# bxlab/bx-python

Measured on AMD Instinct MI355X. Metric: M overlap-queries/s at 100M x 10M intervals (count-only), higher is better.
Workload: dtype int32

## Files before the change

### bx-python_amd/csrc/count_dense.hpp

```cpp
#pragma once
#include "offset_cells.hpp"

namespace bxmi {

constexpr int BD_UNIT_LOG2 = 19;
constexpr int BD_RSHIFT = 19;
constexpr int BD_MARGIN = 8192;
constexpr int BD_MAX_F = 6;
constexpr int BD_MAX_SHIFT = 19;
constexpr int BD_OV_MAX = 32704;
constexpr int BD_TABLE_FROM_FIRST = 2, BD_TABLE_FROM_LAST = 6;
constexpr int BD_THREADS = 1024;
constexpr int BD_LONG_SLOTS = 64;
constexpr int BD_LONG_CAP = 320;
constexpr int BD_HDR_QS = 6;

struct BdLayout {
    int nce, ncs;
    int bitsE, bitsS, metaE, metaS, hdr, ov, bytes;
    int ov_cap;
};

__host__ __device__ inline BdLayout bd_layout(int unit_log2)
{
// ... 917 lines not shown
    {
        const int nl = s_nlong < BD_LONG_CAP ? s_nlong : BD_LONG_CAP;
        for (int k = 0; k < nl; k++) {
            const uint2 lr = s_long[k];
            const unsigned first = lr.x, end = lr.x + lr.y;
            const unsigned q0 = first >> 2, nq4 = ((end + 3u) >> 2) - q0;
            for (unsigned q = threadIdx.x; q < nq4; q += BD_THREADS) {
                const unsigned idx4 = q0 + q;
                bd_answer_slot<FMT, QB, EXP, W8>(I, out, idx4, bd_valid_mask(4u * idx4, first, end), reinterpret_cast<const bd_v4u *>(recs)[idx4]);
            }
        }
    }
}

constexpr int BW_MASK_WORDS = 128;
constexpr int BW_PF = 9;
constexpr unsigned BW_IDLE = 0xFFFFFFFFu;
#ifndef BW_EXP
#define BW_EXP 0
#endif
#ifndef BW_B
#define BW_B 64
#endif
#ifndef BS_UNROLL
#define BS_UNROLL 1
#endif

__device__ __forceinline__ unsigned bw_wave_inclusive_sum(unsigned v)
{
    v += (unsigned)__builtin_amdgcn_update_dpp(0, (int)v, 0x111, 0xf, 0xf, false);
    v += (unsigned)__builtin_amdgcn_update_dpp(0, (int)v, 0x112, 0xf, 0xf, false);
    v += (unsigned)__builtin_amdgcn_update_dpp(0, (int)v, 0x114, 0xf, 0xf, false);
    v += (unsigned)__builtin_amdgcn_update_dpp(0, (int)v, 0x118, 0xf, 0xf, false);
    v += (unsigned)__builtin_amdgcn_update_dpp(0, (int)v, 0x142, 0xa, 0xf, false);
    v += (unsigned)__builtin_amdgcn_update_dpp(0, (int)v, 0x143, 0xc, 0xf, false);
    return v;
}

template <bool RAW = false>
__device__ __forceinline__ void bp_count_slot(const BdImage &I, bd_v4u v, unsigned (&c)[4])
{
    const unsigned rec[4] = {v.x, v.y, v.z, v.w};
    unsigned relE[4], relS[4];
    unsigned long long cellE[4], cellS[4];
#pragma unroll
    for (int j = 0; j < 4; j++) {
// ... 170 lines not shown
    } else {
        bd_v2u o;
        o.x = c[0] | (c[1] << 16), o.y = c[2] | (c[3] << 16);
        reinterpret_cast<bd_v2u *>(out)[idx4] = o;
    }
}

template <bool W8, int DEPTH, bool WIDE = false, int THREADS = BD_THREADS, bool TOT = false>
__global__ __launch_bounds__(THREADS) void bw_search_kernel(const BmSeg *__restrict__ segs, const int4 *__restrict__ items,
                                                               const int *__restrict__ n_items, const unsigned short *__restrict__ unitT, int64_t ntp,
                                                               const unsigned *__restrict__ recs ,
                                                               unsigned short *__restrict__ out , int tile_log2,
                                                               const unsigned *__restrict__ gate, unsigned *__restrict__ xcd_next ,
                                                               unsigned long long *__restrict__ total_slots = nullptr )
{
    if (gate && *gate == 0) return;
    extern __shared__ __attribute__((aligned(16))) int32_t dyn[];
    __shared__ long long s_red[TOT ? THREADS / 64 : 1];
    unsigned long long acc = 0ull;
    int acc_seg = -1;
    constexpr int LONG_CAP = THREADS == BD_THREADS ? BD_LONG_CAP : BD_LONG_CAP / 2;
    constexpr int PF = THREADS == BD_THREADS ? BW_PF : 10;
    __shared__ uint2 s_long[LONG_CAP];
    __shared__ int s_nlong, s_next, s_item_next;
    __shared__ __attribute__((aligned(8))) unsigned s_mask[THREADS / 64][BW_MASK_WORDS];
    const int nit = *n_items;
    const int per_xcd = (nit + 7) >> 3;
    const int xcd = (int)(blockIdx.x & 7);
    const int it_lo = xcd * per_xcd, it_hi = it_lo + per_xcd < nit ? it_lo + per_xcd : nit;
    const int lane = lane_id(), wave = __builtin_amdgcn_readfirstlane((int)(threadIdx.x >> 6));
    unsigned *const wmask = s_mask[wave];
    wmask[lane] = 0u, wmask[64 + lane] = 0u;
    if (threadIdx.x == 0) s_item_next = it_lo + (int)atomicAdd(&xcd_next[xcd], 1u);
    __syncthreads();
    int it = __builtin_amdgcn_readfirstlane(s_item_next);
    __syncthreads();
    const unsigned tile_slots = ((1u << tile_log2) + (unsigned)BM_PAD_ROOM) >> 2;
    while (it < it_hi) {
        const int4 item = items[it];
        const int unit = item.x & 0xffff, t0 = item.y, t1 = item.z;
        const BmSeg &sg = segs[item.x >> 16];
        if (TOT && (item.x >> 16) != acc_seg) {
            if (acc_seg >= 0) {
                block_accumulate_i64((long long)acc, s_red, total_slots + (int64_t)acc_seg * PT_SLOTS + (blockIdx.x & (PT_SLOTS - 1)));
                __syncthreads();
            }
// ... 38 lines not shown
#pragma unroll
            for (int k = 0; k < PF; k++) {
                const int i = k * THREADS + (int)threadIdx.x;
                if (i < n4) reinterpret_cast<bm_v4i *>(dyn)[i] = v[k];
            }
        }
        __syncthreads();
        const int it_nx = __builtin_amdgcn_readfirstlane(s_item_next);
        BdImage I;
        {
            unsigned char *base = reinterpret_cast<unsigned char *>(dyn);
            I.img16 = (lds_u16_p) reinterpret_cast<unsigned short *>(base);
            I.cE = (lds_cell_p) reinterpret_cast<unsigned long long *>(base + LP.cellsE);
            I.cS = (lds_cell_p) reinterpret_cast<unsigned long long *>(base + LP.cellsS);
            const unsigned *hdr = reinterpret_cast<const unsigned *>(base + LP.hdr);
            I.eLo = (int)hdr[0], I.sLo = (int)hdr[1];
            I.bias = I.sLo - I.eLo;
            I.lo = (long long)((unsigned long long)hdr[2] | ((unsigned long long)hdr[3] << 32));
            I.s_ord = sg.ix.s_ord, I.e_sorted = sg.e_sorted;
            I.off_mask = (1u << (g.shift + g.f)) - 1u;
            I.img8 = (lds_u8_p)base;
            I.rshift = g.rshift, I.cell_log2 = cell_log2, I.cell_mask = (1u << cell_log2) - 1u;
        }
        unsigned *const nobody = reinterpret_cast<unsigned *>(reinterpret_cast<unsigned char *>(out) +
                                                              (((size_t)(t0 + (unit * 7 + wave * 64) % (t1 - t0)) + 1) * tile_slots - 1) * (W8 ? 4 : 8));
        unsigned total = 0u, s0 = 0u;
        unsigned delta_c = 0u;
        unsigned win_lo = 0u, win_hi = 0u, win_before = 0u;
        bool live = true;
        auto advance = [&]() -> bool {
            while (tb_next < t1) {
                const int t = tb_next + lane;
                if (((total + 63u) >> 6) < (unsigned)(DEPTH - 1)) asm volatile("s_waitcnt vmcnt(0)" : : : "memory");
                asm volatile("s_waitcnt vmcnt(%2) ; runs %0 %1" : "+v"(a_nx), "+v"(e_nx) : "n"(2 * DEPTH - 2) : "memory");
                const unsigned a = nx_in ? a_nx : 0u, e = nx_in ? e_nx : 0u;
                total = 0u;
                int tn = 0;
                if (lane == 0) tn = atomicAdd(&s_next, B);
                tb_next = t0 + __builtin_amdgcn_readfirstlane(tn);
                load_runs(tb_next);
                unsigned n4 = e > a ? ((e + 3u) >> 2) - (a >> 2) : 0u;
                if (n4 > long_slots) {
                    const int k = atomicAdd(&s_nlong, 1);
                    const unsigned first = ((unsigned)t * tile_slots << 2) + a;
                    if (k < LONG_CAP) {
                        s_long[k] = make_uint2(first, e - a);
                    } else if (TOT) {
                        for (unsigned q = first >> 2; q < ((first + (e - a) + 3u) >> 2); q++) {
                            unsigned c[4];
                            if (WIDE)
                                bo_count_slot<true, THREADS == BD_THREADS>(I, reinterpret_cast<const bd_v4u *>(recs)[q], c);
                            else
                                bp_count_slot<true>(I, reinterpret_cast<const bd_v4u *>(recs)[q], c);
                            acc += (unsigned long long)c[0] + c[1] + c[2] + c[3];
                        }
                    } else {
                        const unsigned esc[4] = {0xFFFFu, 0xFFFFu, 0xFFFFu, 0xFFFFu};
                        for (unsigned q = first >> 2; q < ((first + (e - a) + 3u) >> 2); q++) bw_store_slot<W8>(out, q, esc);
                    }
                    n4 = 0u;
                }
                const unsigned incl = bw_wave_inclusive_sum(n4);
                total = (unsigned)__builtin_amdgcn_readlane((int)incl, 63);
                if (total == 0u) continue;
                const unsigned delta = ((unsigned)t * tile_slots + (a >> 2)) - (incl - n4);
                const bool ne = n4 != 0u;
                const unsigned long long bal = __ballot(ne);
                const unsigned below = __builtin_amdgcn_mbcnt_hi((unsigned)(bal >> 32), __builtin_amdgcn_mbcnt_lo((unsigned)bal, 0u));
                const unsigned dest = ne ? below : 63u - ((unsigned)lane - below);
                delta_c = (unsigned)__builtin_amdgcn_ds_permute((int)(dest << 2), (int)delta);
                if (ne) atomicOr(&wmask[(incl - 1u) >> 5], 1u << ((incl - 1u) & 31u));
                const uint2 w = reinterpret_cast<uint2 *>(wmask)[lane];
                reinterpret_cast<uint2 *>(wmask)[lane] = make_uint2(0u, 0u);
                win_lo = w.x, win_hi = w.y;
                const unsigned ends = (unsigned)__popc(w.x) + (unsigned)__popc(w.y);
                win_before = bw_wave_inclusive_sum(ends) - ends;
                s0 = 0u;
                return true;
            }
            return false;
        };
        bd_v4u ring_v[DEPTH];
        unsigned ring_idx[DEPTH];
        int inflight = 0;
        auto issue = [&](unsigned &idx4, bd_v4u &v) {
            if (live && s0 >= total) live = advance();
            unsigned at = BW_IDLE;
            if (live) {
                const int p = (int)(s0 >> 6);
                const unsigned lo = (unsigned)__builtin_amdgcn_readlane((int)win_lo, p), hi = (unsigned)__builtin_amdgcn_readlane((int)win_hi, p);
                const unsigned before = (unsigned)__builtin_amdgcn_readlane((int)win_before, p);
                const unsigned r = before + __builtin_amdgcn_mbcnt_hi(hi, __builtin_amdgcn_mbcnt_lo(lo, 0u));
                const unsigned dl = (unsigned)__builtin_amdgcn_ds_bpermute((int)(r << 2), (int)delta_c);
                const unsigned s = s0 + (unsigned)lane;
                at = s < total ? dl + s : BW_IDLE;
                s0 += 64u;
            }
            idx4 = at;
            if (live) inflight++;
            bd_issue_load(v, recs, at == BW_IDLE || (BW_EXP & 4) ? 0u : at);
        };
#pragma unroll
        for (int d = 0; d < DEPTH; d++) {
            if (d > 0) bd_dummy_store(reinterpret_cast<unsigned short *>(nobody));
            ring_idx[d] = BW_IDLE;
            bd_issue_load(ring_v[d], recs, 0u);
        }
        for (;;) {
#pragma unroll
            for (int d = 0; d < DEPTH; d++) {
                bd_wait<2 * DEPTH - 2>(ring_v[d]);
                if (__any(ring_idx[d] != BW_IDLE)) {
                    inflight--;
                    if (ring_idx[d] != BW_IDLE) {
                        unsigned c[4];
                        bd_v4u rv = ring_v[d];
                        if (BW_EXP & 4) {
                            const unsigned h = ring_idx[d] * 2654435761u;
                            rv = bd_v4u{(h & 0x3ffffu) | (500u << 18), ((h >> 3) & 0x3ffffu) | (100u << 18), ((h >> 7) & 0x3ffffu) | (900u << 18),
                                        ((h >> 11) & 0x3ffffu) | (300u << 18)};
                        }
// ... 10 lines not shown
                    if (TOT) bd_dummy_store(reinterpret_cast<unsigned short *>(nobody));
                } else {
                    bd_dummy_store(reinterpret_cast<unsigned short *>(nobody));
                }
                issue(ring_idx[d], ring_v[d]);
            }
            if (!live && inflight == 0) break;
        }
#pragma unroll
        for (int d = 0; d < DEPTH; d++) bd_wait<0>(ring_v[d]);
        __syncthreads();
        {
            const int nl = s_nlong < LONG_CAP ? s_nlong : LONG_CAP;
            for (int k = 0; k < nl; k++) {
                const uint2 lr = s_long[k];
                const unsigned q0 = lr.x >> 2, nq4 = ((lr.x + lr.y + 3u) >> 2) - q0;
                for (unsigned q = threadIdx.x; q < nq4; q += THREADS) {
                    unsigned c[4];
                    if (WIDE)
                        bo_count_slot<TOT, THREADS == BD_THREADS>(I, reinterpret_cast<const bd_v4u *>(recs)[q0 + q], c);
                    else
                        bp_count_slot<TOT>(I, reinterpret_cast<const bd_v4u *>(recs)[q0 + q], c);
                    if (TOT) acc += (unsigned long long)c[0] + c[1] + c[2] + c[3];
                    else bw_store_slot<W8>(out, q0 + q, c);
                }
            }
        }
        __syncthreads();
        it = it_nx;
    }
    if (TOT && acc_seg >= 0) block_accumulate_i64((long long)acc, s_red, total_slots + (int64_t)acc_seg * PT_SLOTS + (blockIdx.x & (PT_SLOTS - 1)));
}

__global__ __launch_bounds__(1024) void bs_plan_kernel(const unsigned *__restrict__ bounds , int units, unsigned nq, unsigned chunk,
                                                       int4 *__restrict__ items, int *__restrict__ n_items, const unsigned *__restrict__ gate)
{
    __shared__ int scan_tmp[16];
    if (gate && *gate != 0) return;
    int carry = 0;
    for (int s0 = -1; s0 <= units; s0 += 1024) {
        const int s = s0 + (int)threadIdx.x;
        unsigned lo = 0u, hi = 0u;
        if (s <= units) {
            lo = s < 0 ? 0u : bounds[s];
            hi = s == units ? nq : bounds[s + 1];
        }
        const unsigned n = hi > lo ? hi - lo : 0u;
// ... 179 lines not shown
#pragma unroll
                    for (int j = 0; j < 4; j++) {
                        const bool in = k0 + j >= lo && k0 + j < hi;
                        if (in && c[j] == 0xFFFFu) c[j] = (unsigned)bm_escape_count(sg.ix, sg.e_sorted, g, s[u][j], e[u][j]);
                        if (!in) c[j] = 0u;
                    }
                }
                if (sg.counts) {
                    if (whole[u]) {
                        store_int4(as_global(sg.counts) + 4 * q, (int)c[0], (int)c[1], (int)c[2], (int)c[3]);
                    } else {
#pragma unroll
                        for (int j = 0; j < 4; j++)
                            if (k0 + j >= lo && k0 + j < hi) as_global(sg.counts)[k0 + j] = (int)c[j];
                    }
                }
                acc += (long long)c[0] + c[1] + c[2] + c[3];
            }
        }
        __syncthreads();
        it = it_nx;
    }
    if (total_slots && acc_seg >= 0) block_accumulate_i64(acc, red, total_slots + (int64_t)acc_seg * PT_SLOTS + (blockIdx.x & (PT_SLOTS - 1)));
}

template <int THREADS, int ITEMS, bool PAD, bool W8>
__device__ __forceinline__ void bd_unpermute_tile(const unsigned short *__restrict__ cnt ,
                                                  const unsigned short *__restrict__ slots, const BmSeg *__restrict__ segs,
                                                  const unsigned short *__restrict__ tile_seg,
                                                  unsigned long long *__restrict__ total_slots ,
                                                  const unsigned *__restrict__ gate, const unsigned *__restrict__ tend,
                                                  unsigned long long *__restrict__ fb_dev ,
                                                  unsigned long long *__restrict__ fb_host )
{
    constexpr int TILE = THREADS * ITEMS;
    constexpr int STRIDE = PAD ? TILE + BM_PAD_ROOM : TILE;
    static_assert(ITEMS % 8 == 0, "whole 16-byte vectors of 16-bit counts per thread");
    extern __shared__ __attribute__((aligned(16))) int32_t dyn[];
    if (gate && *gate == 0) return;
    unsigned short *vals = reinterpret_cast<unsigned short *>(dyn);
    __shared__ long long red[THREADS / 64];
    const int64_t tile = blockIdx.x;
    const int seg_id = tile_seg[tile];
    const BmSeg &sg = segs[seg_id];
    const int64_t ltile = tile - sg.tile0;
    if (ltile >= sg.ntiles) return;
// ... 94 lines not shown
    } else {
        for (int k = threadIdx.x; k < n; k += THREADS) {
            unsigned c = W8 ? (unsigned)vals8[slots[k]] : (unsigned)vals[slots[k]];
            if (c == ESC) {
                c = (unsigned)bm_escape_count(ix, e_sorted, g, qs_arr[k], qe_arr[k]);
                wide++;
            }
            if (sg.counts) out[k] = (int)c;
            acc += c;
        }
    }
    if (acc_to) block_accumulate_i64(acc, red, acc_to);
    if (W8 && fb_dev) {
        if (__any(wide != 0u)) {
            unsigned w = wide;
#pragma unroll
            for (int off = 32; off > 0; off >>= 1) w += (unsigned)__shfl_down((int)w, off, 64);
            if (lane_id() == 0 && w) atomicAdd(fb_dev, (unsigned long long)w);
        }
        if (blockIdx.x == 0 && threadIdx.x == 0 && fb_host) *fb_host = __hip_atomic_load(fb_dev, __ATOMIC_RELAXED, __HIP_MEMORY_SCOPE_AGENT);
    }
}

template <int THREADS, int ITEMS, bool PAD = false, bool W8 = false>
__global__ __launch_bounds__(THREADS) void bd_unpermute_kernel(const unsigned short *__restrict__ cnt, const unsigned short *__restrict__ slots,
                                                               const BmSeg *__restrict__ segs, const unsigned short *__restrict__ tile_seg,
                                                               unsigned long long *__restrict__ total_slots, const unsigned *__restrict__ gate,
                                                               const unsigned *__restrict__ tend = nullptr, unsigned long long *__restrict__ fb_dev = nullptr,
                                                               unsigned long long *__restrict__ fb_host = nullptr)
{
    bd_unpermute_tile<THREADS, ITEMS, PAD, W8>(cnt, slots, segs, tile_seg, total_slots, gate, tend, fb_dev, fb_host);
}

}
```

### bx-python_amd/csrc/count_plan.hpp

```cpp
#pragma once
#include <cstddef>
#include <cstdint>
#include <vector>

namespace bxmi {

enum class Stage {
    None,
    Slices,
    Dense,
    Cells,
    OffsetCells,
};
constexpr int N_STAGES = 5;

constexpr int PLAN_NB = 2048;
constexpr int PLAN_GROUP_TILES = 64;
constexpr int PLAN_CHUNK = 65536;
constexpr int PLAN_PAR_CHUNK = 16;
constexpr int PLAN_PAD_ROOM = 4096 + 544;
constexpr int PLAN_PART_Q = 1024;
constexpr int PLAN_SLOTS = 64;
constexpr int PLAN_WALK_THREADS = 1024;
constexpr int PLAN_NBK = 2 * PLAN_NB;
constexpr int PLAN_BOUNDS_ROW = PLAN_NB + 2;
constexpr size_t PLAN_ITEM_BYTES = 16;

struct BmPlanKnobs {
    int64_t bm_variant = -1;
    int64_t sl_flat = 1;
    int64_t bd_chunk = 0;
    int64_t bm_chunk = 0;
    int64_t sl_lanes = 0;
    int64_t bd_w8 = -1;
    int64_t tot_walk = 1;
    int64_t sorted_path = 1;
    int64_t sorted_cells = 1;
    int64_t order_skip = -1;
};

struct BmPlanSegIn {
    int64_t nq = 0;
    int f = 0, shift = 0, stride = 0;
    bool want_counts = true, want_total = false;
    bool bd_blocks = false;
    int bo_state = 0;
    bool w8_off = false;
    int64_t n = 0, span = 1;
    size_t sl_lds = 0;
// ... 26 lines not shown
    int n = 0;
    int64_t nq_all = 0;
    bool wide = false, slices = false, cells = false, fxsub = false;
    bool slices_flat = false;
    bool dense = false;
    int variant = 0;
    int tile_log2 = 14;
    bool pad = false;
    int64_t tile_stride = 0;
    std::vector<BmPlanSegOut> seg;
    int64_t ntp = 0;
    int ngroups = 0;
    int chunk = 0;
    int64_t max_items = 0;
    unsigned sgrid = 0;
    size_t search_lds = 0;
    bool big = false;
    bool any_blocks = false, any_total = false;
    int lanes = -1;
    bool tot_walk = false;
    bool w8_asked = false;
    bool w8 = false;
    bool w8_trip = false;
    bool multi_sorted = false;
    bool order_aware = false;
    bool sorted_on_cells = false;
    unsigned long long order_seen = 0;
    int unsorted_streak = 0;
    bool order_skip = false;
    bool probe_first = false;
    bool order_check = false;
    bool probe_rides = false;
    bool fold_params = false;
    unsigned sorted_chunk = 0;
    size_t sorted_items = 0;
    size_t bounds_bytes = 0;
    size_t seg_bytes = 0, tile_off = 0;
    int n_zero = 0;
    struct Bytes {
        size_t tesc = 0, recs = 0, tend = 0, slots = 0, tbl = 0, runT = 0, unitT = 0, grpcnt = 0, unitcnt = 0, cnt16 = 0, items = 0;
        size_t sl_cnt = 0, sl_loff = 0;
        size_t fx_tbl2 = 0, fx_runT2 = 0, fx_hc = 0, fx_svq = 0, fx_parts = 0, fx_tile_tot = 0, fx_tile_base = 0;
        size_t params = 0, p_slots = 0, bs_plan = 0;
    } bytes;
};

// ... 94 lines not shown
    for (int i = 0; i < n && tot_walk; i++) tot_walk = !in.seg[(size_t)i].want_counts;
    P.tot_walk = tot_walk;

    P.search_lds = slices ? sl_lds : max_stride * 16;
    if (slices_flat && P.search_lds < 4096) P.search_lds = 4096;
    P.big = wide && max_stride * 16 > (size_t)10 * (PLAN_WALK_THREADS / 2) * 16;
    if (slices && !slices_flat) {
        P.lanes = k.sl_lanes < 0 ? 0 : (k.sl_lanes ? (int)k.sl_lanes : (sl_run >= 96 ? 0 : (sl_run >= 40 ? 64 : 16)));
        if (fx && P.lanes == 0) P.lanes = 64;
    }

    if (pad && cells && k.bd_w8 != 0 && !tot_walk) {
        P.w8_asked = true;
        P.w8_trip = (int64_t)in.fb_wide_counts * 64 > in.w8_queries && in.fb_wide_counts > 4096;
        bool narrow = true;
        for (int i = 0; i < n; i++) {
            const BmPlanSegIn &s = in.seg[(size_t)i];
            narrow = narrow && !(s.w8_off || (i == 0 && P.w8_trip)) && s.n * 2048 < s.span * 128;
            if (wide && s.bo_state == 2) narrow = false;
        }
        P.w8 = k.bd_w8 > 0 || narrow;
    }

    bool multi_sorted = n > 1 && !fx && k.sorted_path && k.sorted_cells != 0 && cells && pad;
    for (int i = 0; i < n && multi_sorted; i++) multi_sorted = in.seg[(size_t)i].nq < ((int64_t)1 << 32) - 8;
    P.multi_sorted = multi_sorted;
    P.order_aware = k.sorted_path && (n == 1 || multi_sorted) && !fx;
    P.order_seen = in.order_seen, P.unsorted_streak = in.unsorted_streak;
    bool skip = in.order_skip;
    if (P.order_aware) {
        if ((in.fb_order >> 1) > in.order_seen) {
            P.unsorted_streak = (in.fb_order & 1ull) ? in.unsorted_streak + 1 : 0;
            P.order_seen = in.fb_order >> 1;
            skip = P.unsorted_streak >= 2;
        }
        P.probe_first = in.order_seq == 0 && k.order_skip != 0;
        P.sorted_on_cells = !multi_sorted && cells && pad && k.sorted_cells != 0 && in.seg[0].nq < ((int64_t)1 << 32) - 8;
        P.sorted_chunk = (unsigned)(k.bd_chunk ? k.bd_chunk : (wide ? 1 : 2) * PLAN_CHUNK);
        if (multi_sorted) {
            P.sorted_items = 4;
            for (int i = 0; i < n; i++) P.sorted_items += (size_t)(PLAN_NB >> in.seg[(size_t)i].f) + 4 + (size_t)(in.seg[(size_t)i].nq / P.sorted_chunk);
            P.bounds_bytes = ((size_t)n * PLAN_BOUNDS_ROW * 4 + 16 + 15) & ~(size_t)15;
        } else if (P.sorted_on_cells) {
            const int units = PLAN_NB >> in.seg[0].f;
            P.sorted_items = (size_t)units + 4 + (size_t)(in.seg[0].nq / P.sorted_chunk);
            P.bounds_bytes = (size_t)(units + 2) * 4 + 16;
// ... 42 lines not shown
```

### bx-python_amd/csrc/intervals.hip

```cpp
#include <climits>
#include <vector>
#include <algorithm>
#include <atomic>
#include <condition_variable>
#include <mutex>
#include <thread>
#include <utility>

#include "primitives.hpp"
#include "count_plan.hpp"

#include "count_direct.hpp"
#include "count_parts.hpp"
#include "count_bitmap.hpp"
#include "count_slices.hpp"
#include "find_exchange.hpp"
#include "count_dense.hpp"
#include "find_sorted.hpp"
#include "find_direct.hpp"
#include "find_neighbors.hpp"
#include "cluster.hpp"

namespace bxmi {

// ... 526 lines not shown
    int d = 0;
    while (((Wu + SL_MARGIN) >> d) + 1 > SL_DIR_CELLS) d++;
    g.dshift = d;
    g.ncs = (int32_t)((Wu + SL_MARGIN) >> d) + 1;
    g.nce = (int32_t)(Wu >> d) + 1;
    g.stride = 0;
    *lds_bytes = 2 * ((size_t)h->sl_need[f] + 16) + 2 * (size_t)((g.ncs + 2 + 7) & ~7) + 2 * (size_t)(g.nce + 2 + 8);
    *run_len = (tile << f) / nb_used;
    return g;
}

struct BmLaunch {
    const BmSeg *segs;
    const unsigned short *tile_seg;
    bxmi_ivl *owner;
    int64_t ntp;
    int ngroups, tile_log2;
    size_t search_lds;
    const unsigned *gate;
    bool pad = false;
    bool w8 = false;
    bool wide = false;
    bool big = false;
    bool tot = false;
    unsigned long long *tot_slots = nullptr;
    unsigned *descent = nullptr;
    unsigned *xcd_next = nullptr;
    BmSegChunk par;
    int npar = 0;
    BmParOut par_out;
    int n_segs = 1;
    BmGeom g0;
    unsigned long long order_seq = 0;
};

template <int THREADS, int ITEMS>
static int bm_launch_tiles(const BmLaunch &L, hipStream_t st, bool sub = false)
{
    constexpr int TILE = THREADS * ITEMS;
    bxmi_ivl *h = L.owner;
    auto sort = [&](auto kern, int threads, size_t lds, unsigned *tend, unsigned short *tbl2, unsigned *tesc) {
        return launch_lds(kern, dim3((unsigned)L.ntp), dim3(threads), lds, st, L.segs, L.tile_seg, h->bm_recs.as<unsigned>(), h->bm_slots.as<unsigned short>(),
                          h->bm_tbl.as<unsigned short>(), L.gate, tend, tbl2, L.par, L.npar, L.par_out, tesc);
    };
    if (sub) {
        if (THREADS != 1024 || L.pad) return fail(BXMI_ESTATE, "bm_launch_tiles: half buckets need a 1024-thread shape on packed runs");
// ... 80 lines not shown
static int bd_launch_search(const BmLaunch &L, unsigned grid, Stage fmt, bool blocks, hipStream_t st)
{
    if (fmt == Stage::Cells || fmt == Stage::OffsetCells) {
        if (!L.pad) return fail(BXMI_ESTATE, "bd_launch_search: cell images on packed runs");
        if (L.tot && L.big) return bw_launch_search<false, true, true, true>(L, st);
        if (L.tot) return L.wide ? bw_launch_search<false, true, true>(L, st) : bw_launch_search<false, false, true>(L, st);
        if (L.big) return L.w8 ? bw_launch_search<true, true, false, true>(L, st) : bw_launch_search<false, true, false, true>(L, st);
        if (L.wide) return L.w8 ? bw_launch_search<true, true>(L, st) : bw_launch_search<false, true>(L, st);
        return L.w8 ? bw_launch_search<true, false>(L, st) : bw_launch_search<false, false>(L, st);
    }
    if (fmt == Stage::Slices) return bd_launch_search_t<2, false, 0, 2, false>(L, grid, st);
#ifndef BD_EXP_V
#define BD_EXP_V 0
#endif
    if (L.pad) return blocks ? bd_launch_search_t<0, true, BD_EXP_V, 3, true, true>(L, grid, st) : bd_launch_search_t<0, false, BD_EXP_V, 3, true, true>(L, grid, st);
    return blocks ? bd_launch_search_t<0, true, BD_EXP_V, 4, true>(L, grid, st) : bd_launch_search_t<0, false, BD_EXP_V, 4, true>(L, grid, st);
}

template <int THREADS, int ITEMS>
static int bd_launch_unpermute(const BmLaunch &L, unsigned long long *slots, hipStream_t st)
{
    bxmi_ivl *h = L.owner;
    const bool w8 = L.pad && L.w8;
    auto unpermute = [&](auto kern, size_t count_bytes) {
        return launch_lds(kern, dim3((unsigned)L.ntp), dim3(THREADS), (size_t)(THREADS * ITEMS + (L.pad ? BM_PAD_ROOM : 0)) * count_bytes, st,
                          h->bd_cnt16.as<unsigned short>(), h->bm_slots.as<unsigned short>(), L.segs, L.tile_seg, slots, L.gate,
                          L.pad ? h->bd_tend.as<unsigned>() : nullptr, w8 ? h->bd_fb.as<unsigned long long>() : nullptr, w8 ? h->bd_fb_host : nullptr);
    };
    if (w8) return unpermute(bd_unpermute_kernel<THREADS, ITEMS, true, true>, 1);
    if (L.pad) return unpermute(bd_unpermute_kernel<THREADS, ITEMS, true>, sizeof(unsigned short));
    return unpermute(bd_unpermute_kernel<THREADS, ITEMS, false>, sizeof(unsigned short));
}

static int bs_launch_walk(const BmLaunch &L, const int4 *items, const int *n_items, unsigned long long *tslots, hipStream_t st)
{
    auto walk = [&](auto kern, unsigned grid, unsigned threads) {
        return launch_lds(kern, dim3(grid), dim3(threads), L.search_lds, st, L.segs, items, n_items, tslots, L.gate, L.xcd_next, L.owner->bd_fb_host + 1, L.order_seq);
    };
    if (L.wide && L.big) return walk(bs_walk_kernel<true, BD_THREADS>, 256, BD_THREADS);
    if (L.wide) return walk(bs_walk_kernel<true, BD_THREADS / 2>, 512, BD_THREADS / 2);
    return walk(bs_walk_kernel<false, BD_THREADS>, 256, BD_THREADS);
}

static int bm_launch_plan(const BmLaunch &L, int chunk, hipStream_t st)
{
    bxmi_ivl *h = L.owner;
    if (L.n_segs <= BD_PLAN_SEGS)
        hipLaunchKernelGGL(bd_plan_kernel, dim3(1), dim3(1024), 0, st, h->sl_unitcnt.as<unsigned>(), L.n_segs, L.segs, chunk, h->bm_items.as<int4>() + 1,
                           h->bm_items.as<int>(), L.gate);
    else
        hipLaunchKernelGGL(bm_plan_kernel<2>, dim3(BM_PLAN_BLOCKS), dim3(BM_PLAN_THREADS), 0, st, h->sl_unitcnt.as<unsigned>(), L.ngroups, L.segs, L.tile_seg,
                           chunk, h->bm_items.as<int4>() + 1, h->bm_items.as<int>(), L.gate);
    BXMI_LAUNCH_CHECK();
    return BXMI_OK;
}

static int ensure_feedback(bxmi_ivl *h, hipStream_t st)
{
    if (h->bd_fb_host) return BXMI_OK;
    BXMI_HIP(hipHostMalloc(reinterpret_cast<void **>(&h->bd_fb_host), 64, hipHostMallocDefault));
    memset(h->bd_fb_host, 0, 64);
    BXMI_TRY(h->bd_fb.reserve(64));
    BXMI_HIP(hipMemsetAsync(h->bd_fb.p, 0, 64, st));
    return BXMI_OK;
}

static_assert(PLAN_NB == BM_NB && PLAN_GROUP_TILES == BM_GROUP_TILES && PLAN_CHUNK == BM_CHUNK && PLAN_PAR_CHUNK == BM_PAR_CHUNK &&
                  PLAN_PAD_ROOM == BM_PAD_ROOM && PLAN_PART_Q == BM_PART_Q && PLAN_SLOTS == PT_SLOTS && PLAN_WALK_THREADS == BD_THREADS &&
                  PLAN_NBK == FX_NBK && PLAN_BOUNDS_ROW == BS_BOUNDS_ROW && PLAN_ITEM_BYTES == sizeof(int4),
              "count_plan.hpp and the device headers disagree on a layout constant");

static BmPlanKnobs bm_plan_knobs()
{
    BmPlanKnobs k;
    k.bm_variant = g_opt_bm_variant, k.sl_flat = g_opt_sl_flat, k.bd_chunk = g_opt_bd_chunk, k.bm_chunk = g_opt_bm_chunk, k.sl_lanes = g_opt_sl_lanes;
    k.bd_w8 = g_opt_bd_w8, k.tot_walk = g_opt_tot_walk, k.sorted_path = g_opt_sorted_path, k.sorted_cells = g_opt_sorted_cells;
    k.order_skip = g_opt_order_skip;
    return k;
}

static int bm_reserve(bxmi_ivl *h, const BmPassPlan::Bytes &b)
{
    const struct { DevBuf *buf; size_t bytes; } want[] = {
        {&h->bm_tesc, b.tesc}, {&h->bm_recs, b.recs}, {&h->bd_tend, b.tend}, {&h->bm_slots, b.slots}, {&h->bm_tbl, b.tbl}, {&h->bm_runT, b.runT},
        {&h->bd_unitT, b.unitT}, {&h->bm_grpcnt, b.grpcnt}, {&h->sl_unitcnt, b.unitcnt}, {&h->bd_cnt16, b.cnt16}, {&h->bm_items, b.items},
        {&h->sl_cnt, b.sl_cnt}, {&h->sl_loff, b.sl_loff}, {&h->fx_tbl2, b.fx_tbl2}, {&h->fx_runT2, b.fx_runT2}, {&h->fx_hc, b.fx_hc}, {&h->fx_svq, b.fx_svq},
        {&h->fx_parts, b.fx_parts}, {&h->fx_tile_tot, b.fx_tile_tot}, {&h->fx_tile_base, b.fx_tile_base}, {&h->bm_params, b.params}, {&h->p_slots, b.p_slots}};
    for (const auto &w : want) BXMI_TRY(w.buf->reserve(w.bytes));
    return BXMI_OK;
}

static int bm_set_params(BmLaunch &L, const BmPassPlan &P, const std::vector<BmSeg> &segs, int64_t *const *totals_dev, unsigned long long *slots, hipStream_t st)
// ... 128 lines not shown
            if (seen_descent) {
                h->unsorted_streak = 2, h->order_skip = true;
                bm_plan_set_order_skip(P, true, in.knobs);
            }
        }
        L.order_seq = ++h->order_seq;
    }
    BXMI_TRY(h->bs_plan.reserve(P.bytes.bs_plan));
    if (P.w8_trip) h->w8_off = true;
    if (P.w8) h->w8_queries += P.nq_all;

    unsigned long long *tslots = P.any_total ? slots : nullptr;
    L.owner = h;
    L.gate = P.order_check ? order_word : nullptr;
    L.descent = P.probe_rides ? order_word : nullptr;
    BXMI_TRY(bm_set_params(L, P, segs, totals_dev, slots, st));
    L.ntp = P.ntp, L.ngroups = P.ngroups, L.tile_log2 = P.tile_log2;
    L.search_lds = P.search_lds;
    L.pad = P.pad, L.wide = wide, L.big = P.big, L.w8 = P.w8;
    L.xcd_next = reinterpret_cast<unsigned *>(slots + (size_t)n * PT_SLOTS + 4);
    L.n_segs = n;
    L.g0 = segs[0].g;
    L.tot = P.tot_walk, L.tot_slots = slots;
    if (P.order_check) BXMI_TRY(bm_launch_sorted(L, P, qs, qe, nq, counts, tslots, st));
    if (P.variant == 2)
        BXMI_TRY((bm_launch_tiles<1024, 32>(L, st, P.fxsub)));
    else if (P.variant == 1)
        BXMI_TRY((bm_launch_tiles<1024, 16>(L, st, P.fxsub)));
    else
        BXMI_TRY((bm_launch_tiles<512, 32>(L, st)));
    if (P.tot_walk) {
        hipLaunchKernelGGL(bm_escape_totals_kernel, dim3((unsigned)P.ntp), dim3(1024), 0, st, L.segs, L.tile_seg, h->bm_tesc.as<unsigned>(), P.ntp, P.tile_log2, slots,
                           L.gate);
        BXMI_LAUNCH_CHECK();
    }
    if (P.fxsub) {
        hipLaunchKernelGGL(bm_transpose_kernel<FX_NBK>, dim3((unsigned)P.ngroups, FX_NBK / 64), dim3(256), 0, st, h->fx_tbl2.as<unsigned short>(), L.segs,
                           L.tile_seg, P.tile_log2, h->fx_runT2.as<unsigned>(), P.ntp, (unsigned *)nullptr, L.gate);
        BXMI_LAUNCH_CHECK();
    }
    if (P.dense) {
        hipLaunchKernelGGL(bd_transpose_kernel, dim3((unsigned)P.ngroups, BM_NB / 64), dim3(256), 0, st, h->bm_tbl.as<unsigned short>(), L.segs, L.tile_seg,
                           P.tile_log2, h->bd_unitT.as<unsigned short>(), P.ntp, h->sl_unitcnt.as<unsigned>(), L.gate,
                           P.pad ? h->bd_tend.as<unsigned>() : (const unsigned *)nullptr);
    } else {
        hipLaunchKernelGGL(bm_transpose_kernel<BM_NB>, dim3((unsigned)P.ngroups, BM_NB / 64), dim3(256), 0, st, h->bm_tbl.as<unsigned short>(), L.segs, L.tile_seg,
// ... 979 lines not shown
```

Measured before the change: 149,800.

## Pack walk counts of tile quads contiguously and unpermute by quads

The dense walk now writes per-unit counts of groups of 2 or 4 tiles packed together, using a DPP-computed per-lane shift, instead of at each tile's padded offset. The unpermute kernel processes a quad per block and loads only the used bytes into LDS. In count-only byte mode it can sum the whole region with SAD and skip per-query unpermuting when no escapes remain. This aims to cut padded-region traffic and unpermute launch and work cost, at the price of extra permutes in the walk and a per-slot delta lookup.

```diff
diff --git a/bx-python_amd/csrc/count_dense.hpp b/bx-python_amd/csrc/count_dense.hpp
--- a/bx-python_amd/csrc/count_dense.hpp
+++ b/bx-python_amd/csrc/count_dense.hpp
@@ -963,6 +963,38 @@
 #ifndef BW_B
 #define BW_B 64
 #endif
+#ifndef BM_QUAD
+#define BM_QUAD 4
+#endif
+constexpr int BM_QUAD16 = 2;
+constexpr int BM_QUAD_PAD = 3 * (BM_NB / 2);
+static_assert((BM_QUAD == 2 || BM_QUAD == 4) && BM_GROUP_TILES % BM_QUAD == 0, "a quad never straddles two plan groups");
+static_assert(BM_QUAD_PAD + 32 * BM_QUAD * 4 < BM_PAD_ROOM, "room behind a region's runs for the slots nobody owns");
+
+template <int Q, int J>
+__device__ __forceinline__ unsigned bw_quad_lane(unsigned x)
+{
+    constexpr int ctrl = Q == 4 ? J * 0x55 : (J == 0 ? 0xA0 : 0xF5);
+    return (unsigned)__builtin_amdgcn_update_dpp(0, (int)x, ctrl, 0xf, 0xf, false);
+}
+
+template <int Q>
+__device__ __forceinline__ unsigned bw_quad_shift(unsigned a4, unsigned n4, int lane, unsigned tile_slots)
+{
+    const unsigned j = (unsigned)lane & (unsigned)(Q - 1);
+    const unsigned e4 = a4 + n4;
+    unsigned d = 0u;
+    const unsigned e0 = bw_quad_lane<Q, 0>(e4), a1 = bw_quad_lane<Q, 1>(a4), e1 = bw_quad_lane<Q, 1>(e4);
+    d += j > 0u ? e0 : 0u;
+    d += j > 1u ? e1 : (j < 1u ? a1 : 0u);
+    if (Q == 4) {
+        const unsigned a2 = bw_quad_lane<Q, 2 % Q>(a4), e2 = bw_quad_lane<Q, 2 % Q>(e4), a3 = bw_quad_lane<Q, 3 % Q>(a4);
+        d += j > 2u ? e2 : (j < 2u ? a2 : 0u);
+        d += j < 3u ? a3 : 0u;
+    }
+    return d - j * tile_slots;
+}
+
 #ifndef BS_UNROLL
 #define BS_UNROLL 1
 #endif
@@ -1179,6 +1211,8 @@
     constexpr int LONG_CAP = THREADS == BD_THREADS ? BD_LONG_CAP : BD_LONG_CAP / 2;
     constexpr int PF = THREADS == BD_THREADS ? BW_PF : 10;
     __shared__ uint2 s_long[LONG_CAP];
+    __shared__ unsigned s_long_shift[TOT ? 1 : LONG_CAP];
+    constexpr int Q = W8 ? BM_QUAD : BM_QUAD16;
     __shared__ int s_nlong, s_next, s_item_next;
     __shared__ __attribute__((aligned(8))) unsigned s_mask[THREADS / 64][BW_MASK_WORDS];
     const int nit = *n_items;
@@ -1263,10 +1297,13 @@
             I.img8 = (lds_u8_p)base;
             I.rshift = g.rshift, I.cell_log2 = cell_log2, I.cell_mask = (1u << cell_log2) - 1u;
         }
-        unsigned *const nobody = reinterpret_cast<unsigned *>(reinterpret_cast<unsigned char *>(out) +
-                                                              (((size_t)(t0 + (unit * 7 + wave * 64) % (t1 - t0)) + 1) * tile_slots - 1) * (W8 ? 4 : 8));
+        const size_t nobody_tile = (size_t)(t0 + (unit * 7 + wave * 64) % (t1 - t0));
+        unsigned *const nobody = reinterpret_cast<unsigned *>(
+            reinterpret_cast<unsigned char *>(out) +
+            (TOT ? (nobody_tile + 1) * tile_slots - 1 : (nobody_tile / Q + 1) * Q * tile_slots - 1 - (nobody_tile % Q) * 32) * (W8 ? 4 : 8));
         unsigned total = 0u, s0 = 0u;
         unsigned delta_c = 0u;
+        unsigned shift_c = 0u;
         unsigned win_lo = 0u, win_hi = 0u, win_before = 0u;
         bool live = true;
         auto advance = [&]() -> bool {
@@ -1281,11 +1318,13 @@
                 tb_next = t0 + __builtin_amdgcn_readfirstlane(tn);
                 load_runs(tb_next);
                 unsigned n4 = e > a ? ((e + 3u) >> 2) - (a >> 2) : 0u;
+                const unsigned shift = TOT ? 0u : bw_quad_shift<Q>(a >> 2, n4, lane, tile_slots);
                 if (n4 > long_slots) {
                     const int k = atomicAdd(&s_nlong, 1);
                     const unsigned first = ((unsigned)t * tile_slots << 2) + a;
                     if (k < LONG_CAP) {
                         s_long[k] = make_uint2(first, e - a);
+                        if (!TOT) s_long_shift[k] = shift;
                     } else if (TOT) {
                         for (unsigned q = first >> 2; q < ((first + (e - a) + 3u) >> 2); q++) {
                             unsigned c[4];
@@ -1297,7 +1336,7 @@
                         }
                     } else {
                         const unsigned esc[4] = {0xFFFFu, 0xFFFFu, 0xFFFFu, 0xFFFFu};
-                        for (unsigned q = first >> 2; q < ((first + (e - a) + 3u) >> 2); q++) bw_store_slot<W8>(out, q, esc);
+                        for (unsigned q = first >> 2; q < ((first + (e - a) + 3u) >> 2); q++) bw_store_slot<W8>(out, q + shift, esc);
                     }
                     n4 = 0u;
                 }
@@ -1310,6 +1349,7 @@
                 const unsigned below = __builtin_amdgcn_mbcnt_hi((unsigned)(bal >> 32), __builtin_amdgcn_mbcnt_lo((unsigned)bal, 0u));
                 const unsigned dest = ne ? below : 63u - ((unsigned)lane - below);
                 delta_c = (unsigned)__builtin_amdgcn_ds_permute((int)(dest << 2), (int)delta);
+                if (!TOT) shift_c = (unsigned)__builtin_amdgcn_ds_permute((int)(dest << 2), (int)shift);
                 if (ne) atomicOr(&wmask[(incl - 1u) >> 5], 1u << ((incl - 1u) & 31u));
                 const uint2 w = reinterpret_cast<uint2 *>(wmask)[lane];
                 reinterpret_cast<uint2 *>(wmask)[lane] = make_uint2(0u, 0u);
@@ -1326,7 +1366,7 @@
         int inflight = 0;
         auto issue = [&](unsigned &idx4, bd_v4u &v) {
             if (live && s0 >= total) live = advance();
-            unsigned at = BW_IDLE;
+            unsigned at = BW_IDLE, to = BW_IDLE;
             if (live) {
                 const int p = (int)(s0 >> 6);
                 const unsigned lo = (unsigned)__builtin_amdgcn_readlane((int)win_lo, p), hi = (unsigned)__builtin_amdgcn_readlane((int)win_hi, p);
@@ -1335,9 +1375,14 @@
                 const unsigned dl = (unsigned)__builtin_amdgcn_ds_bpermute((int)(r << 2), (int)delta_c);
                 const unsigned s = s0 + (unsigned)lane;
                 at = s < total ? dl + s : BW_IDLE;
+                to = at;
+                if (!TOT) {
+                    const unsigned sh = (unsigned)__builtin_amdgcn_ds_bpermute((int)(r << 2), (int)shift_c);
+                    to = s < total ? at + sh : BW_IDLE;
+                }
                 s0 += 64u;
             }
-            idx4 = at;
+            idx4 = to;
             if (live) inflight++;
             bd_issue_load(v, recs, at == BW_IDLE || (BW_EXP & 4) ? 0u : at);
         };
@@ -1394,7 +1439,7 @@
                     else
                         bp_count_slot<TOT>(I, reinterpret_cast<const bd_v4u *>(recs)[q0 + q], c);
                     if (TOT) acc += (unsigned long long)c[0] + c[1] + c[2] + c[3];
-                    else bw_store_slot<W8>(out, q0 + q, c);
+                    else bw_store_slot<W8>(out, q0 + q + s_long_shift[k], c);
                 }
             }
         }
@@ -1620,6 +1665,70 @@
         it = it_nx;
     }
     if (total_slots && acc_seg >= 0) block_accumulate_i64(acc, red, total_slots + (int64_t)acc_seg * PT_SLOTS + (blockIdx.x & (PT_SLOTS - 1)));
+}
+
+
+template <int THREADS, int ITEMS, bool W8, typename CountAt>
+__device__ __forceinline__ void bd_unpermute_pick(CountAt count_at, const unsigned short *__restrict__ slots, int n, const IndexDev &ix,
+                                                  const int32_t *__restrict__ e_sorted, const BmGeom &g, const int32_t BX_GLOBAL *__restrict__ qs_arr,
+                                                  const int32_t BX_GLOBAL *__restrict__ qe_arr, int32_t BX_GLOBAL *__restrict__ out, const BmSeg &sg,
+                                                  long long &acc, unsigned &wide)
+{
+    constexpr int TILE = THREADS * ITEMS;
+    constexpr unsigned ESC = W8 ? 0xFFu : 0xFFFFu;
+    if (n == TILE) {
+        const uint2 *l4 = reinterpret_cast<const uint2 *>(slots);
+        int32_t BX_GLOBAL *o4 = out;
+        uint2 sl[ITEMS / 4];
+#pragma unroll
+        for (int j = 0; j < ITEMS / 4; j++) sl[j] = l4[j * THREADS + threadIdx.x];
+#pragma unroll
+        for (int j = 0; j < ITEMS / 4; j++) {
+            unsigned c[4];
+            c[0] = count_at(sl[j].x & 0xffffu), c[1] = count_at(sl[j].x >> 16), c[2] = count_at(sl[j].y & 0xffffu), c[3] = count_at(sl[j].y >> 16);
+            if (c[0] == ESC || c[1] == ESC || c[2] == ESC || c[3] == ESC) {
+                const int64_t k0 = 4 * (int64_t)(j * THREADS + threadIdx.x);
+#pragma unroll
+                for (int u = 0; u < 4; u++)
+                    if (c[u] == ESC) {
+                        c[u] = (unsigned)bm_escape_count(ix, e_sorted, g, qs_arr[k0 + u], qe_arr[k0 + u]);
+                        wide++;
+                    }
+            }
+            if (sg.counts) store_int4(o4 + 4 * (j * THREADS + (int)threadIdx.x), (int)c[0], (int)c[1], (int)c[2], (int)c[3]);
+            acc += (long long)c[0] + c[1] + c[2] + c[3];
+        }
+    } else {
+        for (int k = threadIdx.x; k < n; k += THREADS) {
+            unsigned c = count_at((unsigned)slots[k]);
+            if (c == ESC) {
+                c = (unsigned)bm_escape_count(ix, e_sorted, g, qs_arr[k], qe_arr[k]);
+                wide++;
+            }
+            if (sg.counts) out[k] = (int)c;
+            acc += c;
+        }
+    }
+}
+
+__device__ __forceinline__ void bd_sum_count_bytes(unsigned x, unsigned &sum, unsigned &nff)
+{
+    const unsigned ff = ((x & 0x7F7F7F7Fu) + 0x01010101u) & x & 0x80808080u;
+    const unsigned c = (unsigned)__popc(ff);
+    nff += c;
+    sum += __builtin_amdgcn_sad_u8(x, 0u, 0u) - 255u * c;
+}
+
+__device__ __forceinline__ void bd_count_width_feedback(unsigned wide, unsigned long long *__restrict__ fb_dev, unsigned long long *__restrict__ fb_host)
+{
+    if (!fb_dev) return;
+    if (__any(wide != 0u)) {
+        unsigned w = wide;
+#pragma unroll
+        for (int off = 32; off > 0; off >>= 1) w += (unsigned)__shfl_down((int)w, off, 64);
+        if (lane_id() == 0 && w) atomicAdd(fb_dev, (unsigned long long)w);
+    }
+    if (blockIdx.x == 0 && threadIdx.x == 0 && fb_host) *fb_host = __hip_atomic_load(fb_dev, __ATOMIC_RELAXED, __HIP_MEMORY_SCOPE_AGENT);
 }
 
 template <int THREADS, int ITEMS, bool PAD, bool W8>
@@ -1760,14 +1869,135 @@
     }
 }
 
-template <int THREADS, int ITEMS, bool PAD = false, bool W8 = false>
+template <int THREADS, int ITEMS, bool W8, int Q>
+__device__ __forceinline__ void bd_unpermute_quad(const unsigned short *__restrict__ cnt , const unsigned short *__restrict__ slots,
+                                                  const unsigned short *__restrict__ tbl ,
+                                                  const BmSeg *__restrict__ segs, const unsigned short *__restrict__ tile_seg,
+                                                  unsigned long long *__restrict__ total_slots, const unsigned *__restrict__ gate,
+                                                  const unsigned *__restrict__ tend, unsigned long long *__restrict__ fb_dev,
+                                                  unsigned long long *__restrict__ fb_host)
+{
+    constexpr int TILE = THREADS * ITEMS;
+    constexpr int STRIDE = TILE + BM_PAD_ROOM;
+    constexpr int ROOM = TILE + BM_QUAD_PAD;
+    constexpr int CB = W8 ? 1 : 2;
+    static_assert(THREADS >= BM_NB / 2 && ROOM % 16 == 0, "a thread per unit of two buckets and more");
+    extern __shared__ __attribute__((aligned(16))) int32_t dyn[];
+    if (gate && *gate == 0) return;
+    const unsigned short *vals = reinterpret_cast<const unsigned short *>(dyn);
+    const unsigned char *vals8 = reinterpret_cast<const unsigned char *>(dyn);
+    unsigned short *delta = reinterpret_cast<unsigned short *>(reinterpret_cast<unsigned char *>(dyn) + (size_t)Q * ROOM * CB);
+    __shared__ long long red[THREADS / 64];
+    const int64_t tile0 = (int64_t)blockIdx.x * Q;
+    const int seg_id = tile_seg[tile0];
+    const BmSeg &sg = segs[seg_id];
+    const int64_t ltile0 = tile0 - sg.tile0;
+    if (ltile0 >= sg.ntiles) return;
+    const int nlive = sg.ntiles - ltile0 < Q ? (int)(sg.ntiles - ltile0) : Q;
+    const IndexDev ix = sg.ix;
+    const BmGeom g = sg.g;
+    const int32_t *__restrict__ e_sorted = sg.e_sorted;
+    unsigned used[Q], region = 0u;
+    int64_t n_real = 0;
+#pragma unroll
+    for (int j = 0; j < Q; j++) {
+        used[j] = j < nlive ? tend[tile0 + j] : 0u;
+        used[j] = used[j] < (unsigned)ROOM ? used[j] : (unsigned)ROOM;
+        region += used[j];
+        const int64_t nq = sg.nq - (ltile0 + j) * TILE;
+        n_real += j < nlive ? (nq < TILE ? nq : TILE) : 0;
+    }
+    {
+        const int4 *src = reinterpret_cast<const int4 *>(reinterpret_cast<const unsigned char *>(cnt) + (size_t)tile0 * STRIDE * CB);
+        const int n16 = (int)((region * CB + 15u) >> 4);
+        for (int i = threadIdx.x; i < n16; i += THREADS) reinterpret_cast<int4 *>(dyn)[i] = src[i];
+    }
+    unsigned A[Q], E[Q];
+    {
+        const int units = BM_NB >> g.f, u = (int)threadIdx.x;
+#pragma unroll
+        for (int j = 0; j < Q; j++) {
+            A[j] = E[j] = 0u;
+            if (u < units && j < nlive) {
+                const unsigned short *row = tbl + (tile0 + j) * BM_NB;
+                A[j] = (unsigned)row[u << g.f] >> 2;
+                E[j] = (u + 1 < units ? (unsigned)row[(u + 1) << g.f] : used[j]) >> 2;
+                E[j] = E[j] < (unsigned)(ROOM / 4) ? E[j] : (unsigned)(ROOM / 4);
+            }
+        }
+    }
+    __syncthreads();
+    if (W8 && !sg.counts) {
+        const int n16 = (int)((region + 15u) >> 4);
+        unsigned sum = 0, nff = 0;
+        for (int i = threadIdx.x; i < n16; i += THREADS) {
+            const int4 v = reinterpret_cast<const int4 *>(dyn)[i];
+            const unsigned w[4] = {(unsigned)v.x, (unsigned)v.y, (unsigned)v.z, (unsigned)v.w};
+#pragma unroll
+            for (int k = 0; k < 4; k++)
+                if (16 * i + 4 * k < (int)region) bd_sum_count_bytes(w[k], sum, nff);
+        }
+        __shared__ unsigned s_tot[2];
+        if (threadIdx.x < 2) s_tot[threadIdx.x] = 0u;
+        __syncthreads();
+#pragma unroll
+        for (int off = 32; off > 0; off >>= 1) {
+            sum += (unsigned)__shfl_down((int)sum, off, 64);
+            nff += (unsigned)__shfl_down((int)nff, off, 64);
+        }
+        if (lane_id() == 0) {
+            atomicAdd(&s_tot[0], sum);
+            atomicAdd(&s_tot[1], nff);
+        }
+        __syncthreads();
+        if (s_tot[1] == region - (unsigned)n_real) {
+            if (total_slots && threadIdx.x == 0 && s_tot[0])
+                atomicAdd(total_slots + (int64_t)seg_id * PT_SLOTS + (tile0 & (PT_SLOTS - 1)), (unsigned long long)s_tot[0]);
+            return;
+        }
+    }
+    unsigned wide = 0;
+    for (int j = 0; j < nlive; j++) {
+        const int64_t tile = tile0 + j, ltile = ltile0 + j;
+        if (j) __syncthreads();
+        {
+            unsigned d = 0u, a = 0u, e = 0u;
+#pragma unroll
+            for (int k = 0; k < Q; k++) {
+                d += k < j ? E[k] : (k > j ? A[k] : 0u);
+                if (k == j) a = A[k], e = E[k];
+            }
+            for (unsigned s = a; s < e; s++) delta[s] = (unsigned short)d;
+        }
+        __syncthreads();
+        const int64_t nq = sg.nq - ltile * TILE;
+        const int n = (int)(nq < TILE ? nq : TILE);
+        long long acc = 0;
+        bd_unpermute_pick<THREADS, ITEMS, W8>(
+            [&](unsigned slot) {
+                const unsigned at = slot + 4u * (unsigned)delta[slot >> 2];
+                return W8 ? (unsigned)vals8[at] : (unsigned)vals[at];
+            },
+            slots + tile * TILE, n, ix, e_sorted, g, as_global(sg.qs) + ltile * TILE, as_global(sg.qe) + ltile * TILE, as_global(sg.counts) + ltile * TILE,
+            sg, acc, wide);
+        if (total_slots) block_accumulate_i64(acc, red, total_slots + (int64_t)seg_id * PT_SLOTS + (tile & (PT_SLOTS - 1)));
+    }
+    if (W8) bd_count_width_feedback(wide, fb_dev, fb_host);
+}
+
+template <int THREADS, int ITEMS, bool PAD = false, bool W8 = false, int QUAD = 0>
 __global__ __launch_bounds__(THREADS) void bd_unpermute_kernel(const unsigned short *__restrict__ cnt, const unsigned short *__restrict__ slots,
                                                                const BmSeg *__restrict__ segs, const unsigned short *__restrict__ tile_seg,
                                                                unsigned long long *__restrict__ total_slots, const unsigned *__restrict__ gate,
                                                                const unsigned *__restrict__ tend = nullptr, unsigned long long *__restrict__ fb_dev = nullptr,
-                                                               unsigned long long *__restrict__ fb_host = nullptr)
-{
-    bd_unpermute_tile<THREADS, ITEMS, PAD, W8>(cnt, slots, segs, tile_seg, total_slots, gate, tend, fb_dev, fb_host);
-}
-
-}
+                                                               unsigned long long *__restrict__ fb_host = nullptr,
+                                                               const unsigned short *__restrict__ tbl = nullptr )
+{
+    static_assert(QUAD == 0 || PAD, "counts by quads come with the padded layout");
+    if constexpr (QUAD != 0)
+        bd_unpermute_quad<THREADS, ITEMS, W8, QUAD>(cnt, slots, tbl, segs, tile_seg, total_slots, gate, tend, fb_dev, fb_host);
+    else
+        bd_unpermute_tile<THREADS, ITEMS, PAD, W8>(cnt, slots, segs, tile_seg, total_slots, gate, tend, fb_dev, fb_host);
+}
+
+}
diff --git a/bx-python_amd/csrc/count_plan.hpp b/bx-python_amd/csrc/count_plan.hpp
--- a/bx-python_amd/csrc/count_plan.hpp
+++ b/bx-python_amd/csrc/count_plan.hpp
@@ -25,6 +25,12 @@
 constexpr int PLAN_NBK = 2 * PLAN_NB;
 constexpr int PLAN_BOUNDS_ROW = PLAN_NB + 2;
 constexpr size_t PLAN_ITEM_BYTES = 16;
+#ifndef BM_QUAD
+#define BM_QUAD 4
+#endif
+constexpr int PLAN_QUAD8 = BM_QUAD;
+constexpr int PLAN_QUAD16 = 2;
+constexpr int PLAN_QUAD_PAD = 3 * (PLAN_NB / 2);
 
 struct BmPlanKnobs {
     int64_t bm_variant = -1;
@@ -97,6 +103,9 @@
     bool w8_asked = false;
     bool w8 = false;
     bool w8_trip = false;
+    int quad = 0;
+    unsigned ugrid = 0;
+    size_t unperm_lds = 0;
     bool multi_sorted = false;
     bool order_aware = false;
     bool sorted_on_cells = false;
@@ -237,6 +246,19 @@
         P.w8 = k.bd_w8 > 0 || narrow;
     }
 
+    if (dense && !fxsub && !tot_walk) {
+        const size_t cb = P.w8 ? 1 : 2;
+        P.quad = cells && pad ? (P.w8 ? PLAN_QUAD8 : PLAN_QUAD16) : 0;
+        if (P.quad) {
+            const size_t room = (size_t)(tile + PLAN_QUAD_PAD);
+            P.ugrid = (unsigned)(ntp / P.quad);
+            P.unperm_lds = (size_t)P.quad * room * cb + room / 4 * 2;
+        } else {
+            P.ugrid = (unsigned)ntp;
+            P.unperm_lds = (size_t)(tile + (pad ? PLAN_PAD_ROOM : 0)) * cb;
+        }
+    }
+
     bool multi_sorted = n > 1 && !fx && k.sorted_path && k.sorted_cells != 0 && cells && pad;
     for (int i = 0; i < n && multi_sorted; i++) multi_sorted = in.seg[(size_t)i].nq < ((int64_t)1 << 32) - 8;
     P.multi_sorted = multi_sorted;
diff --git a/bx-python_amd/csrc/intervals.hip b/bx-python_amd/csrc/intervals.hip
--- a/bx-python_amd/csrc/intervals.hip
+++ b/bx-python_amd/csrc/intervals.hip
@@ -572,6 +572,9 @@
     bool w8 = false;
     bool wide = false;
     bool big = false;
+    int quad = 0;
+    unsigned ugrid = 0;
+    size_t unperm_lds = 0;
     bool tot = false;
     unsigned long long *tot_slots = nullptr;
     unsigned *descent = nullptr;
@@ -698,14 +701,16 @@
 {
     bxmi_ivl *h = L.owner;
     const bool w8 = L.pad && L.w8;
-    auto unpermute = [&](auto kern, size_t count_bytes) {
-        return launch_lds(kern, dim3((unsigned)L.ntp), dim3(THREADS), (size_t)(THREADS * ITEMS + (L.pad ? BM_PAD_ROOM : 0)) * count_bytes, st,
-                          h->bd_cnt16.as<unsigned short>(), h->bm_slots.as<unsigned short>(), L.segs, L.tile_seg, slots, L.gate,
-                          L.pad ? h->bd_tend.as<unsigned>() : nullptr, w8 ? h->bd_fb.as<unsigned long long>() : nullptr, w8 ? h->bd_fb_host : nullptr);
+    auto unpermute = [&](auto kern) {
+        return launch_lds(kern, dim3(L.ugrid), dim3(THREADS), L.unperm_lds, st, h->bd_cnt16.as<unsigned short>(), h->bm_slots.as<unsigned short>(), L.segs,
+                          L.tile_seg, slots, L.gate, L.pad ? h->bd_tend.as<unsigned>() : nullptr, w8 ? h->bd_fb.as<unsigned long long>() : nullptr,
+                          w8 ? h->bd_fb_host : nullptr, L.quad ? h->bm_tbl.as<unsigned short>() : nullptr);
     };
-    if (w8) return unpermute(bd_unpermute_kernel<THREADS, ITEMS, true, true>, 1);
-    if (L.pad) return unpermute(bd_unpermute_kernel<THREADS, ITEMS, true>, sizeof(unsigned short));
-    return unpermute(bd_unpermute_kernel<THREADS, ITEMS, false>, sizeof(unsigned short));
+    if (L.quad && (!L.pad || L.quad != (w8 ? BM_QUAD : BM_QUAD16))) return fail(BXMI_ESTATE, "bd_launch_unpermute: counts by quads the kernels do not have");
+    if (L.quad) return w8 ? unpermute(bd_unpermute_kernel<THREADS, ITEMS, true, true, BM_QUAD>) : unpermute(bd_unpermute_kernel<THREADS, ITEMS, true, false, BM_QUAD16>);
+    if (w8) return unpermute(bd_unpermute_kernel<THREADS, ITEMS, true, true>);
+    if (L.pad) return unpermute(bd_unpermute_kernel<THREADS, ITEMS, true>);
+    return unpermute(bd_unpermute_kernel<THREADS, ITEMS, false>);
 }
 
 static int bs_launch_walk(const BmLaunch &L, const int4 *items, const int *n_items, unsigned long long *tslots, hipStream_t st)
@@ -743,7 +748,8 @@
 
 static_assert(PLAN_NB == BM_NB && PLAN_GROUP_TILES == BM_GROUP_TILES && PLAN_CHUNK == BM_CHUNK && PLAN_PAR_CHUNK == BM_PAR_CHUNK &&
                   PLAN_PAD_ROOM == BM_PAD_ROOM && PLAN_PART_Q == BM_PART_Q && PLAN_SLOTS == PT_SLOTS && PLAN_WALK_THREADS == BD_THREADS &&
-                  PLAN_NBK == FX_NBK && PLAN_BOUNDS_ROW == BS_BOUNDS_ROW && PLAN_ITEM_BYTES == sizeof(int4),
+                  PLAN_NBK == FX_NBK && PLAN_BOUNDS_ROW == BS_BOUNDS_ROW && PLAN_ITEM_BYTES == sizeof(int4) && PLAN_QUAD8 == BM_QUAD &&
+                  PLAN_QUAD16 == BM_QUAD16 && PLAN_QUAD_PAD == BM_QUAD_PAD,
               "count_plan.hpp and the device headers disagree on a layout constant");
 
 static BmPlanKnobs bm_plan_knobs()
@@ -918,6 +924,7 @@
     L.n_segs = n;
     L.g0 = segs[0].g;
     L.tot = P.tot_walk, L.tot_slots = slots;
+    L.quad = P.quad, L.ugrid = P.ugrid, L.unperm_lds = P.unperm_lds;
     if (P.order_check) BXMI_TRY(bm_launch_sorted(L, P, qs, qe, nq, counts, tslots, st));
     if (P.variant == 2)
         BXMI_TRY((bm_launch_tiles<1024, 32>(L, st, P.fxsub)));
```

New measurement: 144,700. 0.966x the previous value.
